# erikszasz/GaussianSplattingRegistration

Hardware: AMD Instinct MI355X
Metric: Gaussians/sec through HEM level + ICP iters/sec, 2x5M-splat pair (higher is better)
Workload: dtype f32 (HEM) / f64 (ICP)

## Files before the change

### __graft_entry__.py

```python
from __future__ import annotations

import os
import shutil
import subprocess
import sys

ROOT = os.path.dirname(os.path.abspath(__file__))
CSRC = os.path.join(ROOT, "gaussiansplattingregistration_amd", "csrc")
LIB = os.path.join(CSRC, "libgsr_hip.so")
HIP_SOURCES = ["hem.hip", "hem_select.hip", "icp.hip", "grid.hip", "voxel.hip", "model.hip", "comm.hip", "features.hip", "fgr.hip", "raster.hip", "fuse.hip", "fuse_multi.hip", "posegraph.hip", "clean.hip", "orient.hip", "harmonize.hip", "photo.hip", "warp.hip", "d2d.hip", "imgloss.hip", "covgrad.hip"]
HEADERS = ["gsr_common.h", "gsr_oneshot.h", "gsr_math.h", "gsr_fold.h", "gsr_normals.h", "gsr_solve.h", "gsr_features.h", "gsr_test_hooks.h", "gsr_prims.h", "gsr_posegraph.h", "gsr_colorsolve.h", "gsr_grid.h", "gsr_clean_args.h", "gsr_orient.h", "gsr_fuse_dev.h", "gsr_fuse_args.h", "gsr_model_arrays.h", "gsr_warp.h", "gsr_d2d.h", "gsr_ssim_window.h", "gsr_covbuild.h", "hem_device.h", "hem_select.h",
           "hem_ctx.h", "hem_part_level.h", "hem_level_run.h", os.path.join("..", "..", "include", "gsr_hip.h")]
HIPCC_FLAGS = ["--offload-arch=gfx950", "-O3", "-std=c++17", "-fPIC", "-ffp-contract=off", "-Wall",
               "-Wno-unused-function", "-Wno-unused-result"]
EXTRA_FLAGS = {"hem_select.hip": ["-mllvm", "-disable-machine-licm"]}


def _hipcc() -> str:
    for cand in (shutil.which("hipcc"), "/opt/rocm/bin/hipcc"):
        if cand and os.path.exists(cand):
            return cand
    raise RuntimeError("hipcc not found: cannot build the gfx950 HIP extension")


def _stale(target: str, deps) -> bool:
    if not os.path.exists(target):
        return True
    t = os.path.getmtime(target)
    return any(os.path.getmtime(d) > t for d in deps if os.path.exists(d))


def build_hip(force: bool = False, verbose: bool = False) -> str:
    if os.environ.get("GSR_HIP_LIB"):
        return os.environ["GSR_HIP_LIB"]
    hdrs = [os.path.join(CSRC, h) for h in HEADERS]
    srcs = [os.path.join(CSRC, s) for s in HIP_SOURCES]
    if not force and not _stale(LIB, srcs + hdrs):
        return LIB
    hipcc = _hipcc()
    objs, procs = [], []
    for s in HIP_SOURCES:
        src = os.path.join(CSRC, s)
        obj = os.path.join(CSRC, s.replace(".hip", ".o"))
        objs.append(obj)
        if force or _stale(obj, [src] + hdrs):
            cmd = [hipcc] + HIPCC_FLAGS + EXTRA_FLAGS.get(s, []) + ["-c", src, "-o", obj]
            if verbose:
                print(" ".join(cmd), flush=True)
            procs.append((cmd, subprocess.Popen(cmd, stdout=subprocess.PIPE, stderr=subprocess.STDOUT, text=True)))
    for cmd, p in procs:
        out, _ = p.communicate()
        if p.returncode != 0:
            raise RuntimeError("hipcc failed:\n" + " ".join(cmd) + "\n" + out)
        if verbose and out.strip():
            print(out)
    if force or procs or _stale(LIB, objs):
        cmd = [hipcc, "--offload-arch=gfx950", "-shared", "-fPIC"] + objs + ["-o", LIB]
        r = subprocess.run(cmd, stdout=subprocess.PIPE, stderr=subprocess.STDOUT, text=True)
        if r.returncode != 0:
            raise RuntimeError("link failed:\n" + r.stdout)
    return LIB


def build() -> None:
    build_hip()
    subprocess.check_call(["make", "-C", os.path.join(ROOT, "oracle"), "oracle"], stdout=subprocess.DEVNULL)
    if os.path.isdir("/root/reference/src/cpp_ext"):
        ref_dir = os.path.join(ROOT, "oracle", "_ref")
# ... 42 lines not shown
```

### gaussiansplattingregistration_amd/csrc/hem_select.h

```cpp
#pragma once
#include "hem_device.h"

namespace gsr {

struct ParentRec;
struct SelectArgs {
    const float4* A;
    const float4* geo;
    const float* Rs;
    const unsigned* plist;
    const unsigned* porder;
    int xcd;
    const int* nheavy;
    int own_lo, own_hi;
    const int* cellStart;
    const float4* Ac;
    const int* cellStartC;
    const int* cellStartI;
    const double* logtab;
    const int* irank;
    const unsigned* ipos;
    int n_irr;
    int ell;
    const GridParams* gp;
// ... 45 lines not shown
    float ey, ez;
    int rows;
};
static_assert(sizeof(ParentRec) == 160, "ParentRec is fetched as 40 dwords");

__device__ __forceinline__ float fast_sqrt(float x) { return __builtin_amdgcn_sqrtf(x); }

__device__ __forceinline__ int mbcnt64(unsigned long long mask, int base) {
    return (int)__builtin_amdgcn_mbcnt_hi((unsigned)(mask >> 32), __builtin_amdgcn_mbcnt_lo((unsigned)mask, (unsigned)base));
}
__device__ __forceinline__ unsigned long long uniform64(unsigned long long v) {
    return ((unsigned long long)(unsigned)__builtin_amdgcn_readfirstlane((int)(v >> 32)) << 32) |
           (unsigned)__builtin_amdgcn_readfirstlane((int)v);
}
__device__ __forceinline__ int wave_incl_scan(int v) {
    v += __builtin_amdgcn_update_dpp(0, v, 0x111, 0xf, 0xf, false);
    v += __builtin_amdgcn_update_dpp(0, v, 0x112, 0xf, 0xf, false);
    v += __builtin_amdgcn_update_dpp(0, v, 0x114, 0xf, 0xf, false);
    v += __builtin_amdgcn_update_dpp(0, v, 0x118, 0xf, 0xf, false);
    v += __builtin_amdgcn_update_dpp(0, v, 0x142, 0xa, 0xf, false);
    v += __builtin_amdgcn_update_dpp(0, v, 0x143, 0xc, 0xf, false);
    return v;
}

#ifdef GSR_SELECT_PROFILE
extern __device__ unsigned long long g_sel_prof[1024 * 16];
#define SEL_PROF_T(var) const unsigned long long var = __builtin_amdgcn_s_memtime()
#define SEL_PROF_ADD(slot, t0, lane) do { if ((lane) == 0) atomicAdd(&g_sel_prof[(blockIdx.x & 1023u) * 16 + (slot)], __builtin_amdgcn_s_memtime() - (t0)); } while (0)
#define SEL_PROF_CNT(slot, v, lane) do { if ((lane) == 0) atomicAdd(&g_sel_prof[(blockIdx.x & 1023u) * 16 + (slot)], (unsigned long long)(v)); } while (0)
#else
#define SEL_PROF_T(var)
#define SEL_PROF_ADD(slot, t0, lane)
#define SEL_PROF_CNT(slot, v, lane)
#endif

__device__ __forceinline__ bool kl_gate_rejects(float s2, float det_c, float det_p, float inv_det_p, float thr, const double* logtab,
                                                float* lf_out = nullptr, bool* exact_out = nullptr) {
    const float qf = det_c * inv_det_p;
    const float lf = __builtin_amdgcn_logf(qf) * 0.6931471805599453f;
    const float kf = 0.5f * (s2 - lf);
    const float margin = 1e-6f * (1.0f + fabsf(lf) + fabsf(s2));
    bool reject = kf > thr;
    const bool need_exact = !(qf >= 4.0f * FLT_MIN && qf <= 0.25f * FLT_MAX) || !(fabsf(s2) <= FLT_MAX) || !(fabsf(kf - thr) > margin);
    if (need_exact) {
        const float k = 0.5f * (s2 - glibc_logf_tab(det_c / det_p, logtab));
        reject = k > thr;
    }
    if (lf_out) *lf_out = lf;
    if (exact_out) *exact_out = need_exact;
    return reject;
}


template <bool IRR>
__device__ __forceinline__ void select_row_span(const SelectArgs& a, const GridParams& g, const f3& pm, const EllClip& ec, bool clip,
                                                float Ra2, int x0, int x1, int ry, int rz, int& s, int& len) {
    const bool edge = ry == 0 || ry == g.gy - 1 || rz == 0 || rz == g.gz - 1;
    const float ylo = ry == 0 ? -FLT_MAX : g.oy + ry * g.c - g.slack, yhi = ry == g.gy - 1 ? FLT_MAX : g.oy + (ry + 1) * g.c + g.slack;
    const float zlo = rz == 0 ? -FLT_MAX : g.oz + rz * g.c - g.slack, zhi = rz == g.gz - 1 ? FLT_MAX : g.oz + (rz + 1) * g.c + g.slack;
    const float dy = fmaxf(0.0f, fmaxf(ylo - pm.y, pm.y - yhi));
    const float dz = fmaxf(0.0f, fmaxf(zlo - pm.z, pm.z - zhi));
    const float rem = Ra2 - dy * dy - dz * dz;
    if (rem >= 0.0f) {
        const float hx = fast_sqrt(rem) * 1.00001f + g.slack;
        float lo = -hx, hi = hx;
        if (clip && !edge) {
            const float cy = 0.5f * (ylo + yhi) - pm.y, cz = 0.5f * (zlo + zhi) - pm.z;
            const float hy = 0.5f * (yhi - ylo), hz = 0.5f * (zhi - zlo);
            const float sc = fast_sqrt(fmaxf(0.0f, ec.k11 * cy * cy + 2.0f * ec.k12 * cy * cz + ec.k22 * cz * cz));
            const float smin = fmaxf(0.0f, sc * 0.999f - ec.kr * fast_sqrt(hy * hy + hz * hz));
            const float rem2 = ec.T - smin * smin;
            if (rem2 < 0.0f) {
                lo = 1.0f; hi = -1.0f;
            } else {
                const float w = fast_sqrt(rem2 * ec.im00) * 1.001f;
                const float t1 = ec.m01 * cy, t2 = ec.m02 * cz;
                const float xc = -(t1 + t2) * ec.im00;
                const float dl = (fabsf(ec.m01) * hy + fabsf(ec.m02) * hz) * ec.im00 * 1.001f;
                const float pad = g.slack + 1e-5f * fabsf(xc) + 1e-6f * (fabsf(t1) + fabsf(t2)) * ec.im00;
                lo = fmaxf(lo, xc - dl - w - pad);
                hi = fminf(hi, xc + dl + w + pad);
            }
        }
        if (lo <= hi) {
            int xa = cell_of(pm.x + lo, g.ox, g.inv_c, g.gx), xb = cell_of(pm.x + hi, g.ox, g.inv_c, g.gx);
            xa = xa < x0 ? x0 : xa;
            xb = xb > x1 ? x1 : xb;
            const int rowbase = (rz * g.gy + ry) * g.gx;
            int e;
            if (IRR) { s = a.cellStartI[rowbase + xa]; e = a.cellStartI[rowbase + xb + 1]; }
            else { s = a.cellStartC[rowbase + xa]; e = a.cellStartC[rowbase + xb + 1]; }
            len = e - s;
        }
    }
}

__device__ __forceinline__ void make_filter(const s6& Mf, float det_p, float kldThr, int ell, bool parent_regular, ParentRec& pr) {
    EllClip ec;
    ec.on = 0.0f; ec.k11 = ec.k12 = ec.k22 = ec.kr = ec.im00 = ec.m01 = ec.m02 = 0.0f; ec.T = __builtin_inff();
    pr.white = 0.0f;
    pr.u00 = pr.u01 = pr.u02 = pr.u11 = pr.u12 = pr.u22 = 0.0f;
    pr.T1 = __builtin_inff();
    pr.ey = pr.ez = __builtin_inff();
    const double thr2 = 2.0 * (double)kldThr;
    if (parent_regular && thr2 >= 0.0 && thr2 < 1e30) {
        const double m00 = Mf.e00, m01 = Mf.e01, m02 = Mf.e02, m11 = Mf.e11, m12 = Mf.e12, m22 = Mf.e22;
        double detM;
        const bool finite = fabs(m00) < 1e30 && fabs(m01) < 1e30 && fabs(m02) < 1e30 && fabs(m11) < 1e30 && fabs(m12) < 1e30 && fabs(m22) < 1e30;
        if (finite && spd_det64(m00, m01, m02, m11, m12, m22, detM)) {
            const double trM = m00 + m11 + m22;
            const double e2 = (m00 * m11 - m01 * m01) + (m00 * m22 - m02 * m02) + (m11 * m22 - m12 * m12);
            const double K = trM * e2 / detM * 1.000001;
            const double u = 5.9604644775390625e-8;
            const double theta = 6.1 * u * K + 2.0 * u;
            const double G = -(log(detM) + log((double)det_p)) + 2e-6;
            if (theta <= 0.25 && fabs(G) <= 1.0) {
                const double smin = (thr2 * (1.0 + 2.0 * u) + G + (double)GSR_DET_TOL + 3.2 * theta / (1.0 - theta) + 4e-5) / (1.0 - theta);
                const double T1 = smin * (1.0 + theta) * (1.0 + theta) * (1.0 + 1e-5);
                if (T1 > 0.0 && T1 < 1e30) {
                    const double u00 = sqrt(m00), u01 = m01 / u00, u02 = m02 / u00;
                    const double t11 = m11 - u01 * u01, u11 = sqrt(t11), u12 = (m12 - u01 * u02) / u11;
                    const double t22 = m22 - u02 * u02 - u12 * u12, u22 = sqrt(t22);
                    if (t11 > 0.0 && t22 > 0.0) {
                        pr.u00 = (float)u00; pr.u01 = (float)u01; pr.u02 = (float)u02; pr.u11 = (float)u11; pr.u12 = (float)u12; pr.u22 = (float)u22;
                        pr.T1 = (float)(T1 * (1.0 + 2.0 * u));
                        pr.white = 1.0f;
                        if (ell) {
                            const double Tc = T1 * (1.0 + theta) * (1.0 + theta) * (1.0 + 1e-4);
                            const double fk = 1.0 - 4.0 * theta - 2e-3;
                            const double im00 = 1.0 / m00;
                            const double k11 = (m11 - m01 * m01 * im00) * fk, k12 = (m12 - m01 * m02 * im00) * fk, k22 = (m22 - m02 * m02 * im00) * fk;
                            ec.k11 = (float)k11; ec.k12 = (float)k12; ec.k22 = (float)k22;
                            ec.kr = (float)(sqrt((k11 + k22) / fk) * 1.001);
                            ec.im00 = (float)(im00 * (1.0 + 4.0 * u));
                            ec.m01 = (float)m01; ec.m02 = (float)m02;
                            ec.T = (float)(Tc * (1.0 + 2.0 * u));
                            const bool ok = fk > 0.5 && k11 > 0.0 && k22 > 0.0 && k11 * k22 > k12 * k12 && ec.kr < FLT_MAX && ec.im00 < FLT_MAX && ec.T < FLT_MAX;
                            ec.on = ok ? 1.0f : 0.0f;
                            pr.ey = (float)(sqrt(fmax(0.0, Tc * (m00 * m22 - m02 * m02) / detM)) * 1.001);
                            pr.ez = (float)(sqrt(fmax(0.0, Tc * (m00 * m11 - m01 * m01) / detM)) * 1.001);
                        }
                    }
                }
            }
        }
// ... 25 lines not shown
```

### gaussiansplattingregistration_amd/csrc/hem_select.hip

```cpp
#include "hem_select.h"

namespace gsr {

#ifdef GSR_SELECT_PROFILE
__device__ unsigned long long g_sel_prof[1024 * 16];
#endif
struct __attribute__((aligned(16))) ParLds {
    float4 r0;
    float4 r1;
    float4 r2;
    float4 r3;
    float R2;
    int js;
    int64_t base;
};
static_assert(sizeof(ParLds) == 80, "ParLds is read as four float4 and two 8-byte words");

#define SEL_Q3CAP 128
struct Q3 {
    unsigned *j, *rel;
    float *d2, *cd, *op, *det;
    int h, n;
};

__device__ __forceinline__ void select_stage3(const SelectArgs& a, const ParLds* par, int lane, int cnt, Q3& q3) {
    if (lane < cnt) {
        const int k = (q3.h + lane) & (SEL_Q3CAP - 1);
        const unsigned e = q3.j[k];
        const ParLds* pl = par + (e >> SEL_TAG_SHIFT);
        const float distanceDiff = sqrtf(q3.d2[k]);
        const float cdiff = sqrtf(q3.cd[k]);
        const float distWeight = expf(-distanceDiff * distanceDiff / a.tau2);
        const float colorInfluence = expf(-cdiff * cdiff / a.tau2);
        const float L = distWeight * q3.op[k] * colorInfluence * sqrtf(q3.det[k]);
        const int64_t dst = pl->base + (int64_t)q3.rel[k];
        a.pair_child[dst] = e & SEL_TAG_MASK;
        a.pair_wl[dst] = pl->r3.z * ref_clamp(L, FLT_MIN, 1e8f);
    }
    q3.h = (q3.h + cnt) & (SEL_Q3CAP - 1);
    q3.n -= cnt;
}

template <int MODE>
__device__ __forceinline__ void select_stage2(const SelectArgs& a, const ParLds* par, int lane, int cnt, const unsigned* q, int qh,
                                              unsigned& count_v, Q3& q3) {
    SEL_PROF_T(tp2);
    SEL_PROF_CNT(8, 1, lane); SEL_PROF_CNT(9, cnt, lane);
    bool acc = false;
    unsigned e = 0u;
    int k = 0;
    float d2 = 0.0f, cdiff = 0.0f, op = 0.0f, det_c = 0.0f;
    if (lane < cnt) {
        e = q[(qh + lane) & (SEL_QCAP - 1)];
        const int j = (int)(e & SEL_TAG_MASK);
        k = (int)(e >> SEL_TAG_SHIFT);
        const ParLds* pl = par + k;
        const float4 p0 = pl->r0, p1 = pl->r1;
        const float R2 = pl->R2;
        const float4* row = a.geo + 4 * (int64_t)j;
        float4 ca = row[0], cb = row[1], cc = row[2], cd = row[3];
        asm volatile("" : "+v"(ca.x), "+v"(ca.y), "+v"(ca.z), "+v"(ca.w), "+v"(cb.x), "+v"(cb.y), "+v"(cb.z), "+v"(cb.w),
                          "+v"(cc.x), "+v"(cc.y), "+v"(cc.z), "+v"(cc.w), "+v"(cd.x), "+v"(cd.y), "+v"(cd.z), "+v"(cd.w));
        const f3 cm = {ca.x, ca.y, ca.z};
        const f3 ccol = {cc.z, cc.w, cd.x};
        const f3 pm = {p0.x, p0.y, p0.z}, pcol = {p0.w, p1.x, p1.y};
        const f3 d = sub3(cm, pm);
        d2 = dot3(d, d);
        const f3 dc = sub3(ccol, pcol);
        cdiff = dot3(dc, dc);
        if (d2 < R2 && !(cdiff > a.colorThr2)) {
            const float4 p2 = pl->r2, p3 = pl->r3;
            const s6 ccov = {cb.x, cb.y, cb.z, cb.w, cc.x, cc.y};
            const s6 pinv = {p1.z, p1.w, p2.x, p2.y, p2.z, p2.w};
            det_c = cd.w;
            op = cd.y;
            const float smd = dot3(d, mul6(pinv, d));
            const float tr = trace_prod6(pinv, ccov);
            const float s2 = smd + tr - 3.0f;
            if (!kl_gate_rejects(s2, det_c, p3.x, p3.y, a.kldThr, a.logtab)) {
                const bool child_is_parent = (__float_as_uint(ca.w) & 1u) != 0u;
                acc = !(child_is_parent && j != pl->js);
            }
        }
    }
    const unsigned long long m = __ballot(acc);
    const int na = __popcll(m);
    SEL_PROF_CNT(15, na, lane);
    if (na == 0) { SEL_PROF_ADD(2, tp2, lane); return; }
    const int k_lo = __builtin_amdgcn_readfirstlane(k);
    const int k_hi = __builtin_amdgcn_readlane(k, __builtin_amdgcn_readfirstlane(cnt - 1));
    unsigned rel = 0u;
#pragma unroll
    for (int kk = 0; kk < SEL_NP; ++kk) {
        if (kk < k_lo || kk > k_hi) continue;
        const unsigned long long mk = __ballot(acc && k == kk);
        const unsigned ck = (unsigned)__builtin_amdgcn_readlane((int)count_v, kk);
        if (acc && k == kk) rel = ck + (unsigned)mbcnt64(mk, 0);
        if (lane == kk) count_v += (unsigned)__popcll(mk);
    }
    if (MODE == SEL_COUNT) { SEL_PROF_ADD(2, tp2, lane); return; }
    if (acc) {
        const int t = mbcnt64(m, q3.h + q3.n) & (SEL_Q3CAP - 1);
        q3.j[t] = e; q3.rel[t] = rel; q3.d2[t] = d2; q3.cd[t] = cdiff; q3.op[t] = op; q3.det[t] = det_c;
    }
    q3.n += na;
    __builtin_amdgcn_wave_barrier();
    if (q3.n >= 64) select_stage3(a, par, lane, 64, q3);
    __builtin_amdgcn_wave_barrier();
    SEL_PROF_ADD(2, tp2, lane);
}

__global__ __launch_bounds__(256) void k_parent_prep(int P, const unsigned* __restrict__ plist, const float4* __restrict__ geo,
                                                     const float* __restrict__ Rs, float kldThr, int ell, ParentRec* __restrict__ prec) {
    __shared__ ParentRec s_pr[4][64];
    const int lane = threadIdx.x & 63, wv = threadIdx.x >> 6;
    for (int base = blockIdx.x * blockDim.x + (threadIdx.x & ~63); base < P; base += gridDim.x * blockDim.x) {
        const int p = base + lane;
        if (p < P) {
        ParentRec pr;
        pr.js = (int)plist[p];
        const float4* prow = geo + 4 * (int64_t)pr.js;
        const float4 pa = prow[0], pb = prow[1], pc = prow[2], pd = prow[3];
        pr.pm = {pa.x, pa.y, pa.z};
        pr.det_p = pd.w;
        pr.inv_det_p = 1.0f / pd.w;
        const s6 pcov = {pb.x, pb.y, pb.z, pb.w, pc.x, pc.y};
        pr.pcol = {pc.z, pc.w, pd.x};
        pr.pweight = pd.z;
        pr.pinv = inverse6(pcov, pr.det_p);
        pr.R = Rs[pr.js];
        pr.R2 = pr.R * pr.R;
        make_filter(pr.pinv, pr.det_p, kldThr, ell, (__float_as_uint(pa.w) & 2u) != 0u, pr);
        const bool pm_finite = fabsf(pr.pm.x) <= FLT_MAX && fabsf(pr.pm.y) <= FLT_MAX && fabsf(pr.pm.z) <= FLT_MAX;
        pr.active = (pr.R2 > 0.0f && pm_finite) ? 1 : 0;
        pr.selfq = (pr.active && (__float_as_uint(pa.w) & 2u)) ? 1 : 0;
        pr.rows = 0;
        s_pr[wv][lane] = pr;
        }
        __builtin_amdgcn_wave_barrier();
        const int nrec = P - base < 64 ? P - base : 64;
        const float4* src = reinterpret_cast<const float4*>(s_pr[wv]);
        float4* dst = reinterpret_cast<float4*>(prec + base);
        for (int t = lane; t < nrec * (int)(sizeof(ParentRec) / 16); t += 64) dst[t] = src[t];
        __builtin_amdgcn_wave_barrier();
    }
}

template <int MODE, bool IRR>
__device__ __forceinline__ void select_scan(const SelectArgs& a, const GridParams& g, const ParentRec& pr, const ParLds* par, unsigned ktag,
                                            const float (&vc)[11], int lane, unsigned long long* bits, unsigned* q, int& qh, int& qn, unsigned& count_v,
                                            Q3& q3, unsigned& cum, unsigned lo, unsigned hi, const int2* rl, int lcnt) {
    const f3 pm = pr.pm;
    const EllClip& ec = pr.ec;
    const bool listed = rl != nullptr;
    bool clip = false;
    int x0 = 0, x1 = 0, y0 = 0, z0 = 0, ny = 1, nrows = lcnt;
    float Ra2 = 0.0f;
    if (!listed) {
        int vz;
        asm volatile("v_mov_b32 %0, 0" : "=v"(vz));
        const auto uni = [vz](int v) { return __builtin_amdgcn_readfirstlane(v + vz); };
        const auto unif = [vz](float v) { return __builtin_bit_cast(float, __builtin_amdgcn_readfirstlane(__builtin_bit_cast(int, v) + vz)); };
        const float Ra = unif(fabsf(pr.R) * 1.00001f + g.slack);
        clip = !IRR && ec.on != 0.0f;
        const float Ry = clip ? fminf(Ra, pr.ey + g.slack) : Ra, Rz = clip ? fminf(Ra, pr.ez + g.slack) : Ra;
        x0 = uni(cell_of(pm.x - Ra, g.ox, g.inv_c, g.gx)); x1 = uni(cell_of(pm.x + Ra, g.ox, g.inv_c, g.gx));
        y0 = uni(cell_of(pm.y - Ry, g.oy, g.inv_c, g.gy));
        const int y1 = uni(cell_of(pm.y + Ry, g.oy, g.inv_c, g.gy));
        z0 = uni(cell_of(pm.z - Rz, g.oz, g.inv_c, g.gz));
        const int z1 = uni(cell_of(pm.z + Rz, g.oz, g.inv_c, g.gz));
        ny = y1 - y0 + 1;
        nrows = ny * (z1 - z0 + 1);
        Ra2 = unif(Ra * Ra);
    }
    const bool white = !IRR && pr.white != 0.0f;
    SEL_PROF_CNT(10, nrows, lane);
    for (int rb = 0; rb < nrows; rb += 64) {
        SEL_PROF_T(tpr);
        SEL_PROF_CNT(11, 1, lane);
        const int r = rb + lane;
        int s = 0, len = 0;
        if (r < nrows) {
            if (listed) { const int2 e = rl[r]; s = e.x; len = e.y; }
            else select_row_span<IRR>(a, g, pm, ec, clip, Ra2, x0, x1, y0 + r % ny, z0 + r / ny, s, len);
        }
        len = len > 0 ? len : 0;
        const unsigned long long nz_m = __ballot(len > 0);
        if (nz_m == 0ull) continue;
        const int incl = wave_incl_scan(len);
        const int pre = incl - len;
        const int total = __builtin_amdgcn_readlane(incl, 63);
        const unsigned cum0 = cum;
        cum += (unsigned)total;
        if (hi <= cum0 || lo >= cum) continue;
        const int b_lo = lo > cum0 ? (int)(lo - cum0) : 0;
        const int b_hi = hi - cum0 < (unsigned)total ? (int)(hi - cum0) : total;
        const int nrb = __popcll(nz_m);
        const int below = mbcnt64(nz_m, 0);
        const int dst = len > 0 ? below : nrb + (lane - below);
        const int delta = __builtin_amdgcn_ds_permute(dst << 2, s - pre);
        SEL_PROF_ADD(1, tpr, lane);
        SEL_PROF_CNT(12, nrb, lane); SEL_PROF_CNT(13, total, lane);
        for (int seg0 = b_lo; seg0 < b_hi; seg0 += SEL_MCAP) {
            const int rel = pre - seg0;
            const bool mine = len > 0 && rel >= 0 && rel < SEL_MCAP;
            if (mine) atomicOr(&bits[rel >> 6], 1ull << (rel & 63));
            int rows_before = __popcll(__ballot(len > 0 && rel < 0));
            __builtin_amdgcn_wave_barrier();
            const int seg_end = b_hi < seg0 + SEL_MCAP ? b_hi : seg0 + SEL_MCAP;
            for (int t0 = seg0; t0 < seg_end; t0 += 64 * SEL_U) {
                SEL_PROF_CNT(14, 1, lane);
                SEL_PROF_T(tps);
                float4 ca[SEL_U];
                int jj[SEL_U];
                int left[SEL_U];
#pragma unroll
                for (int u = 0; u < SEL_U; ++u) {
                    const int c0 = t0 + 64 * u;
                    const unsigned long long word = uniform64(bits[(c0 - seg0) >> 6]);
                    const int row = mbcnt64(word >> 1, rows_before - 1 + (int)(word & 1ull));
                    rows_before += __popcll(word);
                    left[u] = seg_end - c0;
                    const int k = c0 + lane + __builtin_amdgcn_ds_bpermute(row << 2, delta);
                    if (IRR) { jj[u] = lane < left[u] ? (int)a.ipos[k] : pr.js; ca[u] = a.A[jj[u]]; }
                    else { jj[u] = k; ca[u] = a.Ac[k]; }
                }
#pragma unroll
                for (int u = 0; u < SEL_U; ++u) {
                    if (left[u] <= 0) continue;
                    const f3 cm = {ca[u].x, ca[u].y, ca[u].z};
                    bool in;
                    if (white) {
                        in = !(white_smd(vc, cm.x, cm.y, cm.z) > vc[9]);
                    } else {
                        const f3 dq = sub3(pm, cm);
                        in = dot3(dq, dq) < pr.R2;
                    }
                    if (!IRR) {
                        in = in && (__float_as_uint(ca[u].w) & 2u);
                        jj[u] = (int)(__float_as_uint(ca[u].w) >> 2);
                    } else {
                        in = in && (!(__float_as_uint(ca[u].w) & 1u) || jj[u] == pr.js);
                    }
                    in = in && lane < left[u];
                    const unsigned long long m = __ballot(in);
                    if (m == 0ull) continue;
                    if (in) q[mbcnt64(m, qh + qn) & (SEL_QCAP - 1)] = (unsigned)jj[u] | ktag;
                    qn += __popcll(m);
                }
                __builtin_amdgcn_wave_barrier();
                SEL_PROF_ADD(4, tps, lane);
                while (qn >= 64) {
                    select_stage2<MODE>(a, par, lane, 64, q, qh, count_v, q3);
                    qh = (qh + 64) & (SEL_QCAP - 1);
                    qn -= 64;
                }
                __builtin_amdgcn_wave_barrier();
            }
            if (mine) bits[rel >> 6] = 0ull;
            __builtin_amdgcn_wave_barrier();
        }
    }
}

__device__ __forceinline__ void select_fill_par(const SelectArgs& a, int p, int64_t base, ParLds* slot) {
    const float4* r = reinterpret_cast<const float4*>(a.prec + p);
    const float4 r0 = r[0], r1 = r[1], r2 = r[2], r3 = r[3];
    slot->r0 = r0; slot->r1 = r1; slot->r2 = r2; slot->r3 = r3;
    slot->R2 = a.prec[p].R2; slot->js = a.prec[p].js; slot->base = base;
}

template <int MODE>
__device__ __forceinline__ void select_parent(const SelectArgs& a, const GridParams& g, int p, int k, unsigned lo, unsigned hi, int lane,
                                              const ParLds* par, unsigned* q, int& qh, int& qn, unsigned long long* bits, unsigned& count_v, Q3& q3) {
    SEL_PROF_T(tp0);
    ParentRec pr;
    {
        typedef unsigned u16v __attribute__((ext_vector_type(16)));
        typedef unsigned u8v __attribute__((ext_vector_type(8)));
        u16v w0, w1; u8v w2;
        const ParentRec* rp = a.prec + p;
        asm volatile("s_load_dwordx16 %0, %3, 0x0\n\ts_load_dwordx16 %1, %3, 0x40\n\ts_load_dwordx8 %2, %3, 0x80\n\ts_waitcnt lgkmcnt(0)"
                     : "=&s"(w0), "=&s"(w1), "=&s"(w2) : "s"(rp) : "memory");
        unsigned raw[40];
        static_assert(sizeof(raw) == sizeof(ParentRec), "the three scalar loads cover the record");
#pragma unroll
        for (int i = 0; i < 16; ++i) { raw[i] = w0[i]; raw[16 + i] = w1[i]; }
#pragma unroll
        for (int i = 0; i < 8; ++i) raw[32 + i] = w2[i];
        __builtin_memcpy(&pr, raw, sizeof(pr));
    }
    float vc[11];
    {
        const float src[11] = {pr.pm.x, pr.pm.y, pr.pm.z, pr.u00, pr.u01, pr.u02, pr.u11, pr.u12, pr.u22, pr.T1, 0.0f};
#pragma unroll
        for (int i = 0; i < 11; ++i) asm volatile("v_mov_b32 %0, %1" : "=v"(vc[i]) : "s"(src[i]));
    }
    const unsigned ktag = (unsigned)k << SEL_TAG_SHIFT;
    unsigned cum = 0;
    if (pr.selfq) {
        cum = 1u;
        if (lo == 0u) {
            if (lane == 0) q[(qh + qn) & (SEL_QCAP - 1)] = (unsigned)pr.js | ktag;
            qn += 1;
        }
        __builtin_amdgcn_wave_barrier();
        if (qn >= 64) {
            select_stage2<MODE>(a, par, lane, 64, q, qh, count_v, q3);
            qh = (qh + 64) & (SEL_QCAP - 1);
            qn -= 64;
        }
    }
    if (pr.active) {
        const int cA = pr.rows & 0xff, cB = (pr.rows >> 8) & 0xff;
        const int2* rlp = (a.rowlist != nullptr && pr.rows < 0) ? a.rowlist + (int64_t)p * (2 * SEL_ROWS) : nullptr;
        select_scan<MODE, false>(a, g, pr, par, ktag, vc, lane, bits, q, qh, qn, count_v, q3, cum, lo, hi,
                                 rlp != nullptr && cA <= SEL_ROWS ? rlp : nullptr, cA);
        if (a.n_irr > 0) select_scan<MODE, true>(a, g, pr, par, ktag, vc, lane, bits, q, qh, qn, count_v, q3, cum, lo, hi,
                                                 rlp != nullptr && cB <= SEL_ROWS ? rlp + SEL_ROWS : nullptr, cB);
    }
    SEL_PROF_ADD(0, tp0, lane);
    SEL_PROF_CNT(7, 1, lane);
}

template <int MODE>
__device__ __forceinline__ void select_flush(const SelectArgs& a, const ParLds* par, int lane, const unsigned* q, int& qh, int& qn,
                                             unsigned& count_v, Q3& q3) {
    while (qn > 0) {
        const int c = qn < 64 ? qn : 64;
        select_stage2<MODE>(a, par, lane, c, q, qh, count_v, q3);
        qh = (qh + c) & (SEL_QCAP - 1);
        qn -= c;
    }
    SEL_PROF_T(tp3);
    if ((MODE == SEL_FILL || MODE == SEL_SPARSE) && q3.n > 0) select_stage3(a, par, lane, q3.n, q3);
    SEL_PROF_ADD(3, tp3, lane);
    __builtin_amdgcn_wave_barrier();
}

template <int MODE, int WPB, bool QUEUE>
__global__ __launch_bounds__(64 * WPB) void k_select(SelectArgs a) {
    __shared__ unsigned s_q[WPB][SEL_QCAP];
    __shared__ unsigned s_q3u[WPB][2][SEL_Q3CAP];
    __shared__ float s_q3f[WPB][4][SEL_Q3CAP];
    __shared__ unsigned long long s_bits[WPB][SEL_MCAP / 64 + SEL_U];
    __shared__ ParLds s_par[WPB][SEL_NP];
    const int lane = threadIdx.x & 63, wv = __builtin_amdgcn_readfirstlane((int)(threadIdx.x >> 6));
    a.logtab = k_logf_tab;
    if (lane < SEL_MCAP / 64 + SEL_U) s_bits[wv][lane] = 0ull;
    unsigned* q = s_q[wv];
    ParLds* par = s_par[wv];
    Q3 q3 = {s_q3u[wv][0], s_q3u[wv][1], s_q3f[wv][0], s_q3f[wv][1], s_q3f[wv][2], s_q3f[wv][3], 0, 0};
    __builtin_amdgcn_wave_barrier();
    const GridParams g = *a.gp;
    int qh = 0, qn = 0;

    if constexpr (QUEUE) {
        const int n_items = a.hq[0];
        const unsigned part = *a.part_p;
        int item = (int)blockIdx.x * WPB + wv;
        while (item < n_items) {
            const uint2 it = a.hitem[item];
            const int p = __builtin_amdgcn_readfirstlane((int)a.porder[it.x]);
            const unsigned lo = (unsigned)__builtin_amdgcn_readfirstlane((int)(it.y * part));
            const unsigned hi = lo + part > lo ? lo + part : 0xffffffffu;
            int64_t base = 0;
            if (MODE == SEL_SPARSE) base = a.poff[p] + lo;
            if (MODE == SEL_SPARSE && a.cap_pairs && (unsigned long long)base + part > a.cap_pairs) {
                if (lane == 0) { a.part_cnt[item] = 0u; *a.abort_p = 1; }
                int nxt0 = 0;
                if (lane == 0) nxt0 = atomicAdd(&a.hq[1], 1);
                item = __builtin_amdgcn_readfirstlane(nxt0);
                continue;
            }
            if (MODE == SEL_FILL) {
                base = a.poff[p];
                for (int k = a.hfirst[p]; k < item; ++k) base += a.part_cnt[k];
            }
            unsigned count_v = 0u;
            if (lane == 0) select_fill_par(a, p, base, par);
            __builtin_amdgcn_wave_barrier();
            select_parent<MODE>(a, g, p, 0, lo, hi, lane, par, q, qh, qn, s_bits[wv], count_v, q3);
            select_flush<MODE>(a, par, lane, q, qh, qn, count_v, q3);
            if (lane == 0 && (MODE == SEL_COUNT || MODE == SEL_SPARSE)) {
                a.part_cnt[item] = count_v;
                atomicAdd(&a.pcnt[p], count_v);
            }
            int nxt = 0;
            if (lane == 0) nxt = atomicAdd(&a.hq[1], 1);
            item = __builtin_amdgcn_readfirstlane(nxt);
            __builtin_amdgcn_wave_barrier();
        }
    } else {
        SEL_PROF_T(tpk);
        const int np = a.np;
        const int ppb = WPB * np;
        const int nheavy = a.nheavy ? *a.nheavy : 0;
        const int nblk = (a.P + ppb - 1) / ppb;
        const int hb = ((nheavy + ppb - 1) / ppb + 7) & ~7;
        const int bid = block_slot((int)blockIdx.x, nblk, hb < nblk ? hb : nblk, a.xcd);
        if (bid < 0) return;
        const int slot0 = (bid * WPB + wv) * np;
        int p_v = -1;
        if (lane < np) {
            const int slot = slot0 + lane;
            if (slot < a.P && !(a.heavy_blocks > 0 && slot < nheavy)) {
                const int p = a.porder ? (int)a.porder[slot] : slot;
                if (p < a.own_lo || p >= a.own_hi) {
                    if (MODE == SEL_COUNT || MODE == SEL_SPARSE) a.pcnt[p] = 0u;
                } else {
                    const int64_t base = (MODE == SEL_FILL || MODE == SEL_SPARSE) ? a.poff[p] : 0;
                    if (MODE == SEL_SPARSE && a.cap_pairs && (unsigned long long)base + a.pcap[p] > a.cap_pairs) {
                        a.pcnt[p] = 0u; *a.abort_p = 1;
                    } else {
                        p_v = p;
                        select_fill_par(a, p, base, par + lane);
                    }
                }
            }
        }
        unsigned long long todo = __ballot(p_v >= 0);
        unsigned count_v = 0u;
        __builtin_amdgcn_wave_barrier();
        SEL_PROF_ADD(5, tpk, lane);
        while (todo != 0ull) {
            const int k = __builtin_ctzll(todo);
            todo &= todo - 1ull;
            const int p = __builtin_amdgcn_readlane(p_v, k);
            select_parent<MODE>(a, g, p, k, 0u, 0xffffffffu, lane, par, q, qh, qn, s_bits[wv], count_v, q3);
        }
        SEL_PROF_T(tpf);
        select_flush<MODE>(a, par, lane, q, qh, qn, count_v, q3);
        SEL_PROF_ADD(6, tpf, lane);
        if (p_v >= 0 && (MODE == SEL_COUNT || MODE == SEL_SPARSE)) a.pcnt[p_v] = count_v;
    }
}

__global__ __launch_bounds__(256) void k_spans(SelectArgs a) {
    const int sub = threadIdx.x & 15;
    const int p = (int)(((int64_t)blockIdx.x * blockDim.x + threadIdx.x) >> 4);
    if (p >= a.P) return;
    unsigned long long scanned = 0;
    int selfq = 0;
    int nA = 0, nB = 0;
    if (p >= a.own_lo && p < a.own_hi) {
        const GridParams g = *a.gp;
        const float4* rq = reinterpret_cast<const float4*>(a.prec + p);
        float4 q0 = rq[0], q3 = rq[3], q6 = rq[6], q7 = rq[7], q8 = rq[8], q9 = rq[9];
        asm volatile("" : "+v"(q0.x), "+v"(q0.y), "+v"(q0.z), "+v"(q3.w), "+v"(q6.y), "+v"(q6.z), "+v"(q6.w), "+v"(q7.x), "+v"(q7.y), "+v"(q7.z), "+v"(q7.w),
                          "+v"(q8.x), "+v"(q8.y), "+v"(q8.w), "+v"(q9.x), "+v"(q9.y), "+v"(q9.z));
        static_assert(offsetof(ParentRec, R) == 60 && offsetof(ParentRec, ec) == 100 && offsetof(ParentRec, active) == 140 && offsetof(ParentRec, ey) == 148,
                      "k_spans reads the record by offsets");
        const f3 pm = {q0.x, q0.y, q0.z};
        const EllClip ec = {q6.y, q6.z, q6.w, q7.x, q7.y, q7.z, q7.w, q8.x, q8.y};
        struct { float R, ey, ez; int active; } rv = {q3.w, q9.y, q9.z, __float_as_int(q8.w)};
        const auto* rp = &rv;
        selfq = __float_as_int(q9.x);
        const unsigned gsh = (unsigned)(threadIdx.x & 48);
        const auto keep_span = [&](int pass, int s, int len, int& n) {
            const unsigned gm = (unsigned)(__ballot(len > 0) >> gsh) & 0xffffu;
            if (len > 0 && a.rowlist) {
                const int pos = n + __popc(gm & ((1u << sub) - 1u));
                if (pos < SEL_ROWS) a.rowlist[((int64_t)p * 2 + pass) * SEL_ROWS + pos] = make_int2(s, len);
            }
            n += __popc(gm);
        };
        if (rp->active) {
            const float Ra = fabsf(rp->R) * 1.00001f + g.slack;
            const float Ra2 = Ra * Ra;
            const int x0 = cell_of(pm.x - Ra, g.ox, g.inv_c, g.gx), x1 = cell_of(pm.x + Ra, g.ox, g.inv_c, g.gx);
            {
                const bool clip = ec.on != 0.0f;
                const float Ry = clip ? fminf(Ra, rp->ey + g.slack) : Ra, Rz = clip ? fminf(Ra, rp->ez + g.slack) : Ra;
                const int y0 = cell_of(pm.y - Ry, g.oy, g.inv_c, g.gy), y1 = cell_of(pm.y + Ry, g.oy, g.inv_c, g.gy);
                const int z0 = cell_of(pm.z - Rz, g.oz, g.inv_c, g.gz), z1 = cell_of(pm.z + Rz, g.oz, g.inv_c, g.gz);
                const int ny = y1 - y0 + 1, nrows = ny * (z1 - z0 + 1);
                for (int r = sub; r < nrows; r += 16) {
                    int s = 0, len = 0;
                    select_row_span<false>(a, g, pm, ec, clip, Ra2, x0, x1, y0 + r % ny, z0 + r / ny, s, len);
                    scanned += (unsigned long long)(len > 0 ? len : 0);
                    keep_span(0, s, len, nA);
                }
            }
            if (a.n_irr > 0) {
                const int y0 = cell_of(pm.y - Ra, g.oy, g.inv_c, g.gy), y1 = cell_of(pm.y + Ra, g.oy, g.inv_c, g.gy);
                const int z0 = cell_of(pm.z - Ra, g.oz, g.inv_c, g.gz), z1 = cell_of(pm.z + Ra, g.oz, g.inv_c, g.gz);
                const int ny = y1 - y0 + 1, nrows = ny * (z1 - z0 + 1);
                for (int r = sub; r < nrows; r += 16) {
                    int s = 0, len = 0;
                    select_row_span<true>(a, g, pm, ec, false, Ra2, x0, x1, y0 + r % ny, z0 + r / ny, s, len);
                    scanned += (unsigned long long)(len > 0 ? len : 0);
                    keep_span(1, s, len, nB);
                }
            }
        }
    }
    for (int o = 8; o > 0; o >>= 1) scanned += __shfl_xor(scanned, o);
    if (selfq) scanned += 1ull;
    if (sub == 0) {
        a.pcap[p] = (unsigned)(scanned > 0xffffffffull ? 0xffffffffull : scanned);
        if (a.rowlist) const_cast<ParentRec*>(a.prec)[p].rows = (int)(0x80000000u | (unsigned)(nA > SEL_ROWS ? 0xff : nA) | ((unsigned)(nB > SEL_ROWS ? 0xff : nB) << 8));
    }
}

void launch_parent_prep(hipStream_t st, int P, const unsigned* plist, const float4* geo, const float* Rs, float kldThr, int ell, ParentRec* prec) {
    hipLaunchKernelGGL(k_parent_prep, dim3(stride_grid(P)), dim3(256), 0, st, P, plist, geo, Rs, kldThr, ell, prec);
}
void launch_spans(hipStream_t st, const SelectArgs& sa) {
    hipLaunchKernelGGL(k_spans, dim3(ceil_div(sa.P, 16)), dim3(256), 0, st, sa);
}
template <int MODE>
static int32_t launch_select_mode(const SelectArgs& sa, hipStream_t st, hipStream_t aux, hipEvent_t ev_fork, hipEvent_t ev_join) {
    constexpr int WPB = SEL_WPB;
    if (sa.heavy_blocks) {
        GSR_HIP(hipEventRecord(ev_fork, st)); GSR_HIP(hipStreamWaitEvent(aux, ev_fork, 0));
        hipLaunchKernelGGL((k_select<MODE, WPB, true>), dim3(sa.heavy_blocks), dim3(64 * WPB), 0, aux, sa);
        GSR_HIP(hipEventRecord(ev_join, aux));
    }
    hipLaunchKernelGGL((k_select<MODE, WPB, false>), dim3(8 * ceil_div(ceil_div(sa.P, WPB * sa.np), 8)), dim3(64 * WPB), 0, st, sa);
    if (sa.heavy_blocks) GSR_HIP(hipStreamWaitEvent(st, ev_join, 0));
    return GSR_OK;
}
int32_t launch_select(int mode, const SelectArgs& sa, hipStream_t st, hipStream_t aux, hipEvent_t ev_fork, hipEvent_t ev_join) {
    if (mode == SEL_SPARSE) return launch_select_mode<SEL_SPARSE>(sa, st, aux, ev_fork, ev_join);
    if (mode == SEL_COUNT) return launch_select_mode<SEL_COUNT>(sa, st, aux, ev_fork, ev_join);
    return launch_select_mode<SEL_FILL>(sa, st, aux, ev_fork, ev_join);
}
void select_set_attributes() {}
int32_t select_profile(unsigned long long* out16, int32_t reset) {
#ifdef GSR_SELECT_PROFILE
    static unsigned long long h[1024 * 16];
    if (out16) {
        if (hipMemcpyFromSymbol(h, HIP_SYMBOL(g_sel_prof), sizeof(h)) != hipSuccess) return GSR_E_HIP;
        for (int k = 0; k < 16; ++k) { out16[k] = 0; for (int b = 0; b < 1024; ++b) out16[k] += h[b * 16 + k]; }
    }
    if (reset) { memset(h, 0, sizeof(h)); if (hipMemcpyToSymbol(HIP_SYMBOL(g_sel_prof), h, sizeof(h)) != hipSuccess) return GSR_E_HIP; }
    return GSR_OK;
#else
    (void)out16; (void)reset;
    return GSR_E_INVALID;
#endif
}

// ... 2 lines not shown
```

Baseline: 573.7 million.

## Cut selection kernel register pressure by rematerialising cold parent and grid data

The selection kernel no longer keeps the full parent record and grid parameters live in scalar registers across the scan. It reloads the cold fields through targeted scalar loads inside the row loop and reads kernel arguments directly from the kernarg segment by offset. The per-lane count is replaced with a small per-wave npair array. SLP vectorisation is also disabled for this file. The goal is lower SGPR/VGPR pressure and fewer spills, in exchange for repeated scalar loads on each row batch and fragile offset-based inline asm.

```diff
diff --git a/__graft_entry__.py b/__graft_entry__.py
--- a/__graft_entry__.py
+++ b/__graft_entry__.py
@@ -13,7 +13,7 @@
            "hem_ctx.h", "hem_part_level.h", "hem_level_run.h", os.path.join("..", "..", "include", "gsr_hip.h")]
 HIPCC_FLAGS = ["--offload-arch=gfx950", "-O3", "-std=c++17", "-fPIC", "-ffp-contract=off", "-Wall",
                "-Wno-unused-function", "-Wno-unused-result"]
-EXTRA_FLAGS = {"hem_select.hip": ["-mllvm", "-disable-machine-licm"]}
+EXTRA_FLAGS = {"hem_select.hip": ["-mllvm", "-disable-machine-licm", "-fno-slp-vectorize"]}
 
 
 def _hipcc() -> str:
diff --git a/gaussiansplattingregistration_amd/csrc/hem_select.h b/gaussiansplattingregistration_amd/csrc/hem_select.h
--- a/gaussiansplattingregistration_amd/csrc/hem_select.h
+++ b/gaussiansplattingregistration_amd/csrc/hem_select.h
@@ -121,8 +121,7 @@
 }
 
 
-template <bool IRR>
-__device__ __forceinline__ void select_row_span(const SelectArgs& a, const GridParams& g, const f3& pm, const EllClip& ec, bool clip,
+__device__ __forceinline__ void select_row_span(const int* cs, const GridParams& g, const f3& pm, const EllClip& ec, bool clip,
                                                 float Ra2, int x0, int x1, int ry, int rz, int& s, int& len) {
     const bool edge = ry == 0 || ry == g.gy - 1 || rz == 0 || rz == g.gz - 1;
     const float ylo = ry == 0 ? -FLT_MAX : g.oy + ry * g.c - g.slack, yhi = ry == g.gy - 1 ? FLT_MAX : g.oy + (ry + 1) * g.c + g.slack;
@@ -156,10 +155,8 @@
             xa = xa < x0 ? x0 : xa;
             xb = xb > x1 ? x1 : xb;
             const int rowbase = (rz * g.gy + ry) * g.gx;
-            int e;
-            if (IRR) { s = a.cellStartI[rowbase + xa]; e = a.cellStartI[rowbase + xb + 1]; }
-            else { s = a.cellStartC[rowbase + xa]; e = a.cellStartC[rowbase + xb + 1]; }
-            len = e - s;
+            s = cs[rowbase + xa];
+            len = cs[rowbase + xb + 1] - s;
         }
     }
 }
diff --git a/gaussiansplattingregistration_amd/csrc/hem_select.hip b/gaussiansplattingregistration_amd/csrc/hem_select.hip
--- a/gaussiansplattingregistration_amd/csrc/hem_select.hip
+++ b/gaussiansplattingregistration_amd/csrc/hem_select.hip
@@ -43,7 +43,7 @@
 
 template <int MODE>
 __device__ __forceinline__ void select_stage2(const SelectArgs& a, const ParLds* par, int lane, int cnt, const unsigned* q, int qh,
-                                              unsigned& count_v, Q3& q3) {
+                                              unsigned (&npair)[SEL_NP], Q3& q3) {
     SEL_PROF_T(tp2);
     SEL_PROF_CNT(8, 1, lane); SEL_PROF_CNT(9, cnt, lane);
     bool acc = false;
@@ -94,9 +94,8 @@
     for (int kk = 0; kk < SEL_NP; ++kk) {
         if (kk < k_lo || kk > k_hi) continue;
         const unsigned long long mk = __ballot(acc && k == kk);
-        const unsigned ck = (unsigned)__builtin_amdgcn_readlane((int)count_v, kk);
-        if (acc && k == kk) rel = ck + (unsigned)mbcnt64(mk, 0);
-        if (lane == kk) count_v += (unsigned)__popcll(mk);
+        if (acc && k == kk) rel = npair[kk] + (unsigned)mbcnt64(mk, 0);
+        npair[kk] += (unsigned)__popcll(mk);
     }
     if (MODE == SEL_COUNT) { SEL_PROF_ADD(2, tp2, lane); return; }
     if (acc) {
@@ -146,44 +145,88 @@
     }
 }
 
+typedef unsigned sel_u4v __attribute__((ext_vector_type(4)));
+typedef unsigned sel_u8v __attribute__((ext_vector_type(8)));
+struct ParHot { float R2, white; int js, active, selfq, rows; };
+struct ScanCold { f3 pm; float R, ey, ez; EllClip ec; GridParams g; };
+static_assert(offsetof(ParentRec, R) == 60 && offsetof(ParentRec, R2) == 64 && offsetof(ParentRec, u00) == 72 && offsetof(ParentRec, T1) == 96 &&
+              offsetof(ParentRec, ec) == 100 && offsetof(ParentRec, js) == 136 && offsetof(ParentRec, ey) == 148 && offsetof(ParentRec, rows) == 156 &&
+              sizeof(EllClip) == 36 && sizeof(GridParams) == 40 && offsetof(GridParams, gz) == 32,
+              "the selection's scalar loads read the record and the grid by offsets");
+__device__ __forceinline__ float sel_f(unsigned u) { return __builtin_bit_cast(float, u); }
+
+constexpr int SEL_KARG0 = 0;
+template <typename T, int OFF>
+__device__ __forceinline__ T sel_karg() {
+    static_assert(sizeof(T) == 4 || sizeof(T) == 8, "one or two dwords");
+    const auto kp = __builtin_amdgcn_kernarg_segment_ptr();
+    if constexpr (sizeof(T) == 8) {
+        unsigned long long v;
+        asm volatile("s_load_dwordx2 %0, %1, %2\n\ts_waitcnt lgkmcnt(0)" : "=s"(v) : "s"(kp), "n"(OFF));
+        return __builtin_bit_cast(T, v);
+    } else {
+        unsigned v;
+        asm volatile("s_load_dword %0, %1, %2\n\ts_waitcnt lgkmcnt(0)" : "=s"(v) : "s"(kp), "n"(OFF));
+        return __builtin_bit_cast(T, v);
+    }
+}
+#define SEL_KARG(member) sel_karg<decltype(SelectArgs::member), SEL_KARG0 + (int)offsetof(SelectArgs, member)>()
+template <typename... P> struct sel_only_args : std::false_type {};
+template <> struct sel_only_args<SelectArgs> : std::true_type {};
+template <typename... P> constexpr bool sel_kernel_takes_only_args(void (*)(P...)) { return sel_only_args<P...>::value; }
+__device__ __forceinline__ void select_load_cold(const ParentRec* rp, const GridParams* gp, ScanCold& c) {
+    sel_u4v w0; sel_u8v w1, wg;
+    unsigned wR, wT, wgz;
+    unsigned long long we;
+    asm volatile("s_load_dwordx4 %0, %7, 0x0\n\ts_load_dword %1, %7, 0x3c\n\ts_load_dwordx8 %2, %7, 0x64\n\ts_load_dword %3, %7, 0x84\n\t"
+                 "s_load_dwordx2 %4, %7, 0x94\n\ts_load_dwordx8 %5, %8, 0x0\n\ts_load_dword %6, %8, 0x20\n\ts_waitcnt lgkmcnt(0)"
+                 : "=&s"(w0), "=&s"(wR), "=&s"(w1), "=&s"(wT), "=&s"(we), "=&s"(wg), "=&s"(wgz) : "s"(rp), "s"(gp) : "memory");
+    c.pm = {sel_f(w0[0]), sel_f(w0[1]), sel_f(w0[2])};
+    c.R = sel_f(wR);
+    c.ec = {sel_f(w1[0]), sel_f(w1[1]), sel_f(w1[2]), sel_f(w1[3]), sel_f(w1[4]), sel_f(w1[5]), sel_f(w1[6]), sel_f(w1[7]), sel_f(wT)};
+    c.ey = sel_f((unsigned)we); c.ez = sel_f((unsigned)(we >> 32));
+    c.g.ox = sel_f(wg[0]); c.g.oy = sel_f(wg[1]); c.g.oz = sel_f(wg[2]); c.g.c = sel_f(wg[3]); c.g.inv_c = sel_f(wg[4]); c.g.slack = sel_f(wg[5]);
+    c.g.gx = (int)wg[6]; c.g.gy = (int)wg[7]; c.g.gz = (int)wgz; c.g.ncells = 0;
+}
+
 template <int MODE, bool IRR>
-__device__ __forceinline__ void select_scan(const SelectArgs& a, const GridParams& g, const ParentRec& pr, const ParLds* par, unsigned ktag,
-                                            const float (&vc)[11], int lane, unsigned long long* bits, unsigned* q, int& qh, int& qn, unsigned& count_v,
+__device__ __forceinline__ void select_scan(const SelectArgs& a, const ParentRec* rp, const ParHot& pr, const ParLds* par, unsigned ktag,
+                                            const float (&vc)[11], int lane, unsigned long long* bits, unsigned* q, int& qh, int& qn, unsigned (&npair)[SEL_NP],
                                             Q3& q3, unsigned& cum, unsigned lo, unsigned hi, const int2* rl, int lcnt) {
-    const f3 pm = pr.pm;
-    const EllClip& ec = pr.ec;
     const bool listed = rl != nullptr;
-    bool clip = false;
-    int x0 = 0, x1 = 0, y0 = 0, z0 = 0, ny = 1, nrows = lcnt;
-    float Ra2 = 0.0f;
-    if (!listed) {
-        int vz;
-        asm volatile("v_mov_b32 %0, 0" : "=v"(vz));
-        const auto uni = [vz](int v) { return __builtin_amdgcn_readfirstlane(v + vz); };
-        const auto unif = [vz](float v) { return __builtin_bit_cast(float, __builtin_amdgcn_readfirstlane(__builtin_bit_cast(int, v) + vz)); };
-        const float Ra = unif(fabsf(pr.R) * 1.00001f + g.slack);
-        clip = !IRR && ec.on != 0.0f;
-        const float Ry = clip ? fminf(Ra, pr.ey + g.slack) : Ra, Rz = clip ? fminf(Ra, pr.ez + g.slack) : Ra;
-        x0 = uni(cell_of(pm.x - Ra, g.ox, g.inv_c, g.gx)); x1 = uni(cell_of(pm.x + Ra, g.ox, g.inv_c, g.gx));
-        y0 = uni(cell_of(pm.y - Ry, g.oy, g.inv_c, g.gy));
-        const int y1 = uni(cell_of(pm.y + Ry, g.oy, g.inv_c, g.gy));
-        z0 = uni(cell_of(pm.z - Rz, g.oz, g.inv_c, g.gz));
-        const int z1 = uni(cell_of(pm.z + Rz, g.oz, g.inv_c, g.gz));
-        ny = y1 - y0 + 1;
-        nrows = ny * (z1 - z0 + 1);
-        Ra2 = unif(Ra * Ra);
-    }
+    int nrows = listed ? lcnt : 0x40000000;
     const bool white = !IRR && pr.white != 0.0f;
-    SEL_PROF_CNT(10, nrows, lane);
     for (int rb = 0; rb < nrows; rb += 64) {
         SEL_PROF_T(tpr);
         SEL_PROF_CNT(11, 1, lane);
         const int r = rb + lane;
         int s = 0, len = 0;
-        if (r < nrows) {
-            if (listed) { const int2 e = rl[r]; s = e.x; len = e.y; }
-            else select_row_span<IRR>(a, g, pm, ec, clip, Ra2, x0, x1, y0 + r % ny, z0 + r / ny, s, len);
-        }
+        if (listed) {
+            if (r < nrows) { const int2 e = rl[r]; s = e.x; len = e.y; }
+        } else {
+            ScanCold c;
+            select_load_cold(rp, SEL_KARG(gp), c);
+            const int* cs = IRR ? SEL_KARG(cellStartI) : SEL_KARG(cellStartC);
+            const GridParams& g = c.g;
+            const f3 pm = c.pm;
+            int vz;
+            asm volatile("v_mov_b32 %0, 0" : "=v"(vz));
+            const auto uni = [vz](int v) { return __builtin_amdgcn_readfirstlane(v + vz); };
+            const auto unif = [vz](float v) { return __builtin_bit_cast(float, __builtin_amdgcn_readfirstlane(__builtin_bit_cast(int, v) + vz)); };
+            const float Ra = unif(fabsf(c.R) * 1.00001f + g.slack);
+            const bool clip = !IRR && c.ec.on != 0.0f;
+            const float Ry = clip ? fminf(Ra, c.ey + g.slack) : Ra, Rz = clip ? fminf(Ra, c.ez + g.slack) : Ra;
+            const int x0 = uni(cell_of(pm.x - Ra, g.ox, g.inv_c, g.gx)), x1 = uni(cell_of(pm.x + Ra, g.ox, g.inv_c, g.gx));
+            const int y0 = uni(cell_of(pm.y - Ry, g.oy, g.inv_c, g.gy));
+            const int y1 = uni(cell_of(pm.y + Ry, g.oy, g.inv_c, g.gy));
+            const int z0 = uni(cell_of(pm.z - Rz, g.oz, g.inv_c, g.gz));
+            const int z1 = uni(cell_of(pm.z + Rz, g.oz, g.inv_c, g.gz));
+            const int ny = y1 - y0 + 1;
+            nrows = ny * (z1 - z0 + 1);
+            const float Ra2 = unif(Ra * Ra);
+            if (r < nrows) select_row_span(cs, g, pm, c.ec, clip, Ra2, x0, x1, y0 + r % ny, z0 + r / ny, s, len);
+        }
+        if (rb == 0) SEL_PROF_CNT(10, nrows, lane);
         len = len > 0 ? len : 0;
         const unsigned long long nz_m = __ballot(len > 0);
         if (nz_m == 0ull) continue;
@@ -233,6 +276,7 @@
                     if (white) {
                         in = !(white_smd(vc, cm.x, cm.y, cm.z) > vc[9]);
                     } else {
+                        const f3 pm = {vc[0], vc[1], vc[2]};
                         const f3 dq = sub3(pm, cm);
                         in = dot3(dq, dq) < pr.R2;
                     }
@@ -251,7 +295,7 @@
                 __builtin_amdgcn_wave_barrier();
                 SEL_PROF_ADD(4, tps, lane);
                 while (qn >= 64) {
-                    select_stage2<MODE>(a, par, lane, 64, q, qh, count_v, q3);
+                    select_stage2<MODE>(a, par, lane, 64, q, qh, npair, q3);
                     qh = (qh + 64) & (SEL_QCAP - 1);
                     qn -= 64;
                 }
@@ -271,30 +315,23 @@
 }
 
 template <int MODE>
-__device__ __forceinline__ void select_parent(const SelectArgs& a, const GridParams& g, int p, int k, unsigned lo, unsigned hi, int lane,
-                                              const ParLds* par, unsigned* q, int& qh, int& qn, unsigned long long* bits, unsigned& count_v, Q3& q3) {
+__device__ __forceinline__ void select_parent(const SelectArgs& a, int p, int k, unsigned lo, unsigned hi, int lane,
+                                              const ParLds* par, unsigned* q, int& qh, int& qn, unsigned long long* bits, unsigned (&npair)[SEL_NP], Q3& q3) {
     SEL_PROF_T(tp0);
-    ParentRec pr;
+    const ParentRec* rp = SEL_KARG(prec) + p;
+    ParHot pr;
+    float vc[11];
+    vc[10] = 0.0f;
     {
-        typedef unsigned u16v __attribute__((ext_vector_type(16)));
-        typedef unsigned u8v __attribute__((ext_vector_type(8)));
-        u16v w0, w1; u8v w2;
-        const ParentRec* rp = a.prec + p;
-        asm volatile("s_load_dwordx16 %0, %3, 0x0\n\ts_load_dwordx16 %1, %3, 0x40\n\ts_load_dwordx8 %2, %3, 0x80\n\ts_waitcnt lgkmcnt(0)"
-                     : "=&s"(w0), "=&s"(w1), "=&s"(w2) : "s"(rp) : "memory");
-        unsigned raw[40];
-        static_assert(sizeof(raw) == sizeof(ParentRec), "the three scalar loads cover the record");
+        sel_u4v w0; sel_u8v w1, w2;
+        unsigned wT;
+        asm volatile("s_load_dwordx4 %0, %4, 0x0\n\ts_load_dwordx8 %1, %4, 0x40\n\ts_load_dword %2, %4, 0x60\n\ts_load_dwordx8 %3, %4, 0x80\n\ts_waitcnt lgkmcnt(0)"
+                     : "=&s"(w0), "=&s"(w1), "=&s"(wT), "=&s"(w2) : "s"(rp) : "memory");
+        pr.R2 = sel_f(w1[0]); pr.white = sel_f(w1[1]);
+        pr.js = (int)w2[2]; pr.active = (int)w2[3]; pr.selfq = (int)w2[4]; pr.rows = (int)w2[7];
+        const unsigned src[10] = {w0[0], w0[1], w0[2], w1[2], w1[3], w1[4], w1[5], w1[6], w1[7], wT};
 #pragma unroll
-        for (int i = 0; i < 16; ++i) { raw[i] = w0[i]; raw[16 + i] = w1[i]; }
-#pragma unroll
-        for (int i = 0; i < 8; ++i) raw[32 + i] = w2[i];
-        __builtin_memcpy(&pr, raw, sizeof(pr));
-    }
-    float vc[11];
-    {
-        const float src[11] = {pr.pm.x, pr.pm.y, pr.pm.z, pr.u00, pr.u01, pr.u02, pr.u11, pr.u12, pr.u22, pr.T1, 0.0f};
-#pragma unroll
-        for (int i = 0; i < 11; ++i) asm volatile("v_mov_b32 %0, %1" : "=v"(vc[i]) : "s"(src[i]));
+        for (int i = 0; i < 10; ++i) asm volatile("v_mov_b32 %0, %1" : "=v"(vc[i]) : "s"(src[i]));
     }
     const unsigned ktag = (unsigned)k << SEL_TAG_SHIFT;
     unsigned cum = 0;
@@ -306,17 +343,18 @@
         }
         __builtin_amdgcn_wave_barrier();
         if (qn >= 64) {
-            select_stage2<MODE>(a, par, lane, 64, q, qh, count_v, q3);
+            select_stage2<MODE>(a, par, lane, 64, q, qh, npair, q3);
             qh = (qh + 64) & (SEL_QCAP - 1);
             qn -= 64;
         }
     }
     if (pr.active) {
         const int cA = pr.rows & 0xff, cB = (pr.rows >> 8) & 0xff;
-        const int2* rlp = (a.rowlist != nullptr && pr.rows < 0) ? a.rowlist + (int64_t)p * (2 * SEL_ROWS) : nullptr;
-        select_scan<MODE, false>(a, g, pr, par, ktag, vc, lane, bits, q, qh, qn, count_v, q3, cum, lo, hi,
+        int2* const rowlist = SEL_KARG(rowlist);
+        const int2* rlp = (rowlist != nullptr && pr.rows < 0) ? rowlist + (int64_t)p * (2 * SEL_ROWS) : nullptr;
+        select_scan<MODE, false>(a, rp, pr, par, ktag, vc, lane, bits, q, qh, qn, npair, q3, cum, lo, hi,
                                  rlp != nullptr && cA <= SEL_ROWS ? rlp : nullptr, cA);
-        if (a.n_irr > 0) select_scan<MODE, true>(a, g, pr, par, ktag, vc, lane, bits, q, qh, qn, count_v, q3, cum, lo, hi,
+        if (SEL_KARG(n_irr) > 0) select_scan<MODE, true>(a, rp, pr, par, ktag, vc, lane, bits, q, qh, qn, npair, q3, cum, lo, hi,
                                                  rlp != nullptr && cB <= SEL_ROWS ? rlp + SEL_ROWS : nullptr, cB);
     }
     SEL_PROF_ADD(0, tp0, lane);
@@ -325,10 +363,10 @@
 
 template <int MODE>
 __device__ __forceinline__ void select_flush(const SelectArgs& a, const ParLds* par, int lane, const unsigned* q, int& qh, int& qn,
-                                             unsigned& count_v, Q3& q3) {
+                                             unsigned (&npair)[SEL_NP], Q3& q3) {
     while (qn > 0) {
         const int c = qn < 64 ? qn : 64;
-        select_stage2<MODE>(a, par, lane, c, q, qh, count_v, q3);
+        select_stage2<MODE>(a, par, lane, c, q, qh, npair, q3);
         qh = (qh + c) & (SEL_QCAP - 1);
         qn -= c;
     }
@@ -345,6 +383,7 @@
     __shared__ float s_q3f[WPB][4][SEL_Q3CAP];
     __shared__ unsigned long long s_bits[WPB][SEL_MCAP / 64 + SEL_U];
     __shared__ ParLds s_par[WPB][SEL_NP];
+    static_assert(SEL_KARG0 == 0 && sel_kernel_takes_only_args(&k_select<MODE, WPB, QUEUE>), "SEL_KARG reads the argument segment by offsetof(SelectArgs, member)");
     const int lane = threadIdx.x & 63, wv = __builtin_amdgcn_readfirstlane((int)(threadIdx.x >> 6));
     a.logtab = k_logf_tab;
     if (lane < SEL_MCAP / 64 + SEL_U) s_bits[wv][lane] = 0ull;
@@ -352,7 +391,6 @@
     ParLds* par = s_par[wv];
     Q3 q3 = {s_q3u[wv][0], s_q3u[wv][1], s_q3f[wv][0], s_q3f[wv][1], s_q3f[wv][2], s_q3f[wv][3], 0, 0};
     __builtin_amdgcn_wave_barrier();
-    const GridParams g = *a.gp;
     int qh = 0, qn = 0;
 
     if constexpr (QUEUE) {
@@ -360,34 +398,36 @@
         const unsigned part = *a.part_p;
         int item = (int)blockIdx.x * WPB + wv;
         while (item < n_items) {
-            const uint2 it = a.hitem[item];
-            const int p = __builtin_amdgcn_readfirstlane((int)a.porder[it.x]);
+            const uint2 it = SEL_KARG(hitem)[item];
+            const int p = __builtin_amdgcn_readfirstlane((int)SEL_KARG(porder)[it.x]);
             const unsigned lo = (unsigned)__builtin_amdgcn_readfirstlane((int)(it.y * part));
             const unsigned hi = lo + part > lo ? lo + part : 0xffffffffu;
             int64_t base = 0;
-            if (MODE == SEL_SPARSE) base = a.poff[p] + lo;
-            if (MODE == SEL_SPARSE && a.cap_pairs && (unsigned long long)base + part > a.cap_pairs) {
-                if (lane == 0) { a.part_cnt[item] = 0u; *a.abort_p = 1; }
+            if (MODE == SEL_SPARSE) base = SEL_KARG(poff)[p] + lo;
+            const unsigned long long cap_pairs = MODE == SEL_SPARSE ? SEL_KARG(cap_pairs) : 0ull;
+            if (MODE == SEL_SPARSE && cap_pairs && (unsigned long long)base + part > cap_pairs) {
+                if (lane == 0) { SEL_KARG(part_cnt)[item] = 0u; *SEL_KARG(abort_p) = 1; }
                 int nxt0 = 0;
-                if (lane == 0) nxt0 = atomicAdd(&a.hq[1], 1);
+                if (lane == 0) nxt0 = atomicAdd(&SEL_KARG(hq)[1], 1);
                 item = __builtin_amdgcn_readfirstlane(nxt0);
                 continue;
             }
             if (MODE == SEL_FILL) {
-                base = a.poff[p];
-                for (int k = a.hfirst[p]; k < item; ++k) base += a.part_cnt[k];
-            }
-            unsigned count_v = 0u;
+                base = SEL_KARG(poff)[p];
+                const unsigned* part_cnt = SEL_KARG(part_cnt);
+                for (int k = SEL_KARG(hfirst)[p]; k < item; ++k) base += part_cnt[k];
+            }
+            unsigned npair[SEL_NP] = {};
             if (lane == 0) select_fill_par(a, p, base, par);
             __builtin_amdgcn_wave_barrier();
-            select_parent<MODE>(a, g, p, 0, lo, hi, lane, par, q, qh, qn, s_bits[wv], count_v, q3);
-            select_flush<MODE>(a, par, lane, q, qh, qn, count_v, q3);
+            select_parent<MODE>(a, p, 0, lo, hi, lane, par, q, qh, qn, s_bits[wv], npair, q3);
+            select_flush<MODE>(a, par, lane, q, qh, qn, npair, q3);
             if (lane == 0 && (MODE == SEL_COUNT || MODE == SEL_SPARSE)) {
-                a.part_cnt[item] = count_v;
-                atomicAdd(&a.pcnt[p], count_v);
+                SEL_KARG(part_cnt)[item] = npair[0];
+                atomicAdd(&SEL_KARG(pcnt)[p], npair[0]);
             }
             int nxt = 0;
-            if (lane == 0) nxt = atomicAdd(&a.hq[1], 1);
+            if (lane == 0) nxt = atomicAdd(&SEL_KARG(hq)[1], 1);
             item = __builtin_amdgcn_readfirstlane(nxt);
             __builtin_amdgcn_wave_barrier();
         }
@@ -420,19 +460,24 @@
             }
         }
         unsigned long long todo = __ballot(p_v >= 0);
-        unsigned count_v = 0u;
+        unsigned npair[SEL_NP] = {};
         __builtin_amdgcn_wave_barrier();
         SEL_PROF_ADD(5, tpk, lane);
         while (todo != 0ull) {
             const int k = __builtin_ctzll(todo);
             todo &= todo - 1ull;
             const int p = __builtin_amdgcn_readlane(p_v, k);
-            select_parent<MODE>(a, g, p, k, 0u, 0xffffffffu, lane, par, q, qh, qn, s_bits[wv], count_v, q3);
+            select_parent<MODE>(a, p, k, 0u, 0xffffffffu, lane, par, q, qh, qn, s_bits[wv], npair, q3);
         }
         SEL_PROF_T(tpf);
-        select_flush<MODE>(a, par, lane, q, qh, qn, count_v, q3);
+        select_flush<MODE>(a, par, lane, q, qh, qn, npair, q3);
         SEL_PROF_ADD(6, tpf, lane);
-        if (p_v >= 0 && (MODE == SEL_COUNT || MODE == SEL_SPARSE)) a.pcnt[p_v] = count_v;
+        if (p_v >= 0 && (MODE == SEL_COUNT || MODE == SEL_SPARSE)) {
+            unsigned mine = npair[0];
+#pragma unroll
+            for (int kk = 1; kk < SEL_NP; ++kk) mine = lane == kk ? npair[kk] : mine;
+            a.pcnt[p_v] = mine;
+        }
     }
 }
 
@@ -477,7 +522,7 @@
                 const int ny = y1 - y0 + 1, nrows = ny * (z1 - z0 + 1);
                 for (int r = sub; r < nrows; r += 16) {
                     int s = 0, len = 0;
-                    select_row_span<false>(a, g, pm, ec, clip, Ra2, x0, x1, y0 + r % ny, z0 + r / ny, s, len);
+                    select_row_span(a.cellStartC, g, pm, ec, clip, Ra2, x0, x1, y0 + r % ny, z0 + r / ny, s, len);
                     scanned += (unsigned long long)(len > 0 ? len : 0);
                     keep_span(0, s, len, nA);
                 }
@@ -488,7 +533,7 @@
                 const int ny = y1 - y0 + 1, nrows = ny * (z1 - z0 + 1);
                 for (int r = sub; r < nrows; r += 16) {
                     int s = 0, len = 0;
-                    select_row_span<true>(a, g, pm, ec, false, Ra2, x0, x1, y0 + r % ny, z0 + r / ny, s, len);
+                    select_row_span(a.cellStartI, g, pm, ec, false, Ra2, x0, x1, y0 + r % ny, z0 + r / ny, s, len);
                     scanned += (unsigned long long)(len > 0 ? len : 0);
                     keep_span(1, s, len, nB);
                 }
```

Measured after the change: 588.5 million, median of 6. 2.6% higher.
